# penn-graphics-research/claymore

Hardware: AMD Instinct MI355X
Metric: particles*steps/sec (higher is better)
Workload: dtype f32

## Files before the change

claymore_amd/_ffi.py:

```python
import ctypes as C
import os

MPM_OK, MPM_ERR_INVALID, MPM_ERR_DEVICE, MPM_ERR_CAPACITY, MPM_ERR_NONFINITE, MPM_ERR_NOT_READY, MPM_ERR_INTERNAL = range(7)
J_FLUID, FIXED_COROTATED, SAND, NACC = range(4)
MATERIAL_NAMES = {"jfluid": J_FLUID, "fixed_corotated": FIXED_COROTATED, "sand": SAND, "nacc": NACC}


class Config(C.Structure):
    _fields_ = [("domain_bits", C.c_int), ("max_ppc", C.c_int), ("boundary_blocks", C.c_int),
                ("gravity", C.c_float), ("cfl", C.c_float), ("max_blocks", C.c_int64),
                ("grow", C.c_int), ("drop_overflow", C.c_int), ("sync_interval", C.c_int), ("reserved", C.c_int * 3)]


class MaterialParams(C.Structure):
    _fields_ = [("rho", C.c_float), ("volume", C.c_float), ("youngs_modulus", C.c_float),
                ("poisson_ratio", C.c_float), ("bulk", C.c_float), ("gamma", C.c_float),
                ("viscosity", C.c_float), ("beta", C.c_float), ("xi", C.c_float),
                ("cohesion", C.c_float), ("yield_surface", C.c_float), ("msqr", C.c_float),
                ("log_jp0", C.c_float), ("volume_correction", C.c_int), ("hardening_on", C.c_int),
                ("reserved", C.c_int * 5)]


class CollisionObject(C.Structure):
    _fields_ = [("type", C.c_int), ("friction", C.c_float), ("scale", C.c_float), ("dsdt", C.c_float),
                ("trans", C.c_float * 3), ("trans_vel", C.c_float * 3), ("omega", C.c_float * 3),
                ("rot_mat", C.c_float * 9), ("time", C.c_float), ("reserved", C.c_int * 3)]
# ... 12 lines not shown
class Heightfield(C.Structure):
    _fields_ = [("nx", C.c_int), ("nz", C.c_int), ("origin", C.c_float * 2), ("spacing", C.c_float), ("inside_out", C.c_int),
                ("reserved", C.c_int * 6)]


HEIGHTFIELD_MAX_SAMPLES = 4096


class Counts(C.Structure):
    _fields_ = [("particle_blocks", C.c_int), ("neighbor_blocks", C.c_int), ("exterior_blocks", C.c_int),
                ("model_count", C.c_int), ("bins", C.c_int64 * 8), ("particles", C.c_int64 * 8)]


class Diagnostics(C.Structure):
    _fields_ = [("lost_particles", C.c_int64), ("discarded_p2g", C.c_int64), ("overflow_flags", C.c_int),
                ("dropped_particles", C.c_int), ("reserved", C.c_int * 4)]


class Timers(C.Structure):
    _fields_ = [("grid_update_ms", C.c_float), ("g2p2g_ms", C.c_float), ("partition_ms", C.c_float),
                ("halo_ms", C.c_float), ("total_ms", C.c_float), ("reserved", C.c_float * 3)]


_P = C.POINTER
_vp, _i, _f, _sz = C.c_void_p, C.c_int, C.c_float, C.c_size_t
_fp, _ip = _P(C.c_float), _P(C.c_int)

SIGNATURES = {
    "default_config": (_i, [_i, _P(Config)]),
    "default_material": (_i, [_i, _i, _P(MaterialParams)]),
    "create": (_i, [_P(Config), _i, _P(_vp)]),
# ... 114 lines not shown
```

claymore_amd/csrc/claymore_hip.hip:

```cpp
#include <hip/hip_runtime.h>

#include <algorithm>
#include <cmath>
#include <cstdio>
#include <cstdlib>
#include <chrono>
#include <cstring>
#include <string>
#include <vector>

#include "../../include/claymore_amd.h"
#include "mpm_kernels.hpp"
#include "mpm_readout.hpp"
#include "mpm_particle_ids.hpp"

using namespace mpm;

namespace {
constexpr int kHaloWords	 = 128;
constexpr int kStatusBlock = ST_WORDS + kHaloWords + kMaxVelSlots * kMaxVelStride;

struct Partition {
	int* table = nullptr;
	int* keys  = nullptr;
// ... 35 lines not shown
struct mpm_ctx {
	mpm_config cfg {};
	GridCfg g {};
	int device = 0;
	hipStream_t s_compute = nullptr, s_comm = nullptr;
	SubstepEvents ev;
	hipEvent_t ev_comm = nullptr, ev_halo = nullptr;
	hipEvent_t ev_tag0 = nullptr, ev_tag1 = nullptr;
	bool lean_events = false;
	hipEvent_t ev_pending = nullptr;
	hipEvent_t ev_status = nullptr;
	bool grid_preupdated = false;
	bool grid_momentum = false;
	float preupdate_dt	 = 0.f;
	float fuse_dt_once	 = 0.f;
	bool rebuild_cleared = false;
	std::vector<hipEvent_t> ev_ring;
	Partition part[2];
	float* grid[2] = {nullptr, nullptr};
	int rollid	   = 0;
	int pbc = 0, nbc = 0, ebc = 0;
	int pbc_prev = 0;
	std::vector<Model> models;
	int* d_status		  = nullptr;
	int* h_status		  = nullptr;
	unsigned* d_maxvel	  = nullptr;
	float* h_maxvel		  = nullptr;
	double* d_totals	  = nullptr;
	unsigned long long* d_counter = nullptr;
	bool ready = false;
// ... 375 lines not shown
	HIP_TRY(hipStreamSynchronize(s));
	if(pbc > g.cap) return fail(ctx, MPM_ERR_CAPACITY, "Too much active blocks: " + std::to_string(pbc));
	ctx->pbc = pbc;
	if(ctx->cfg.max_blocks <= 0 && (size_t) pbc * 27 > prov) {
		int* keys		  = nullptr;
		const size_t need = std::min(table, (size_t) pbc * 27 + 1);
		HIP_TRY(dalloc(&keys, 3 * need));
		HIP_TRY(hipMemcpyAsync(keys, P.keys, sizeof(int) * 3 * (size_t) pbc, hipMemcpyDeviceToDevice, s));
		HIP_TRY(hipStreamSynchronize(s));
		HIP_TRY(hipFree(P.keys));
		P.keys = keys;
		prov   = need;
		g.cap  = (int) prov;
	}
	HIP_TRY(hipMemcpyAsync(&ctx->d_status[ST_CNT_P], P.count, sizeof(int), hipMemcpyDeviceToDevice, s));
	register_blocks_kernel<0, 1><<<std::max(1u, std::min(4096u, cdiv((size_t) pbc * 8, 256))), 256, 0, s>>>(g, &ctx->d_status[ST_CNT_P], nullptr, &ctx->d_status[ST_CNT_N], &ctx->d_status[ST_PBC], P.table, P.keys, ctx->d_status);
	register_blocks_kernel<-1, 1><<<std::max(1u, std::min(8192u, cdiv((size_t) pbc * 32, 256))), 256, 0, s>>>(g, &ctx->d_status[ST_CNT_P], &ctx->d_status[ST_CNT_N], &ctx->d_status[ST_CNT_E], &ctx->d_status[ST_NBC], P.table, P.keys, ctx->d_status);
	{
		int rc0 = read_status(ctx);
		if(rc0) return rc0;
		rc0 = check_status(ctx);
		if(rc0) return rc0;
		const int ebc0 = ctx->h_status[ST_CNT_P] + ctx->h_status[ST_CNT_N] + ctx->h_status[ST_CNT_E];
		ctx->h_status[ST_EBC] = ebc0;
		ctx->pbc_prev		  = pbc;
		HIP_TRY(hipMemcpyAsync(&ctx->d_status[ST_EBC], &ctx->h_status[ST_EBC], sizeof(int), hipMemcpyHostToDevice, s));
		HIP_TRY(hipMemcpyAsync(&ctx->d_status[ST_PBCPREV], &ctx->pbc_prev, sizeof(int), hipMemcpyHostToDevice, s));
		HIP_TRY(hipMemcpyAsync(P.count, &ctx->h_status[ST_EBC], sizeof(int), hipMemcpyHostToDevice, s));
		HIP_TRY(hipStreamSynchronize(s));
	}
	ctx->nbc = ctx->h_status[ST_NBC];
	ctx->ebc = ctx->h_status[ST_EBC];
// ... 51 lines not shown
		ctx->models[mi].bincount_src = ctx->models[mi].bincount;
		ctx->models[mi].bucketed = (int64_t) ctx->models[mi].n;
		if((size_t) ctx->models[mi].bincount > ctx->models[mi].bin_cap) return fail(ctx, MPM_ERR_CAPACITY, "bin capacity");
	}
	HIP_TRY(hipMemcpyAsync(ctx->part[r].table, P.table, sizeof(int) * table, hipMemcpyDeviceToDevice, s));
	HIP_TRY(hipMemcpyAsync(ctx->part[r].keys, P.keys, sizeof(int) * 3 * (size_t) ctx->ebc, hipMemcpyDeviceToDevice, s));
	HIP_TRY(hipMemcpyAsync(ctx->part[r].count, P.count, sizeof(int), hipMemcpyDeviceToDevice, s));
	HIP_TRY(hipMemsetAsync(ctx->grid[0], 0, sizeof(float) * 256 * (size_t) ctx->nbc, s));
	for(auto& m: ctx->models)
		if(m.n && pbc) rasterize_blocks_kernel<<<pbc, 256, 0, s>>>(g, m.d_xyz, m.list[1], m.size, ctx->part[r].keys, ctx->part[r].table, ctx->grid[0], m.mc.mass, m.v0[0], m.v0[1], m.v0[2]);
	rc = launch_prepare(ctx, r, n, false, r, &ctx->d_status[ST_PBC], ctx->pbc, true, false);
	if(rc) return rc;
	HIP_TRY(hipGetLastError());
	HIP_TRY(hipStreamSynchronize(s));
	ctx->ready		   = true;
	ctx->grid_momentum = true;
	ctx->ids_valid	   = ctx->track_ids;
	return MPM_OK;
}

static CollisionArgs collision_tick(mpm_ctx* ctx, float dt) {
	CollisionArgs a {ctx->collision, collision_pose(ctx->collision, ctx->collision.time)};
	if(ctx->collision_running) ctx->collision.time = ctx->collision.time + dt;
	return a;
}
static ShapeArgs shapes_tick(mpm_ctx* ctx, float dt) {
	ShapeArgs a {};
	const float T = ctx->collision.time;
	a.count		  = ctx->shape_count;
	a.has_field	  = ctx->has_collision ? 1 : 0;
// ... 172 lines not shown
	PrepareModels pm {};
	pm.n = (int) ctx->models.size();
	for(int mi = 0; mi < pm.n; ++mi) {
		Model& m		  = ctx->models[mi];
		pm.list[mi]		  = m.list[list_is_out ? (m.list_in ^ 1) : m.list_in];
		pm.size[mi]		  = m.size;
		pm.row_of[mi]	  = m.row_of;
		pm.binoff_src[mi] = m.binoff[binoff_sel];
		pm.blockinfo[mi]  = m.blockinfo;
		pm.keep[mi]		  = sort && list_is_out ? m.keep : nullptr;
		pm.pairinfo[mi]	  = m.pair ? m.pairinfo[0] : nullptr;
		pm.pairhand[mi]	  = m.pairinfo[1];
	}
	const int nwg = std::max(1, std::min(ctx->g.cap, nblocks_est + nblocks_est / 16 + 64));
	int* pub	  = publish ? ctx->d_status : nullptr;
	if(sort)
		prepare_blocks_kernel<true><<<nwg, 64, 0, ctx->s_compute>>>(ctx->g, pm, pbc_ptr, ctx->part[cur].table, ctx->part[cur].keys, ctx->part[prev].table, pub, ctx->part[cur].count);
	else
		prepare_blocks_kernel<false><<<nwg, 64, 0, ctx->s_compute>>>(ctx->g, pm, pbc_ptr, ctx->part[cur].table, ctx->part[cur].keys, ctx->part[prev].table, pub, ctx->part[cur].count);
	return MPM_OK;
}

static int launch_rebuild_prepare(mpm_ctx* ctx) {
	const int r = ctx->rollid, n = r ^ 1;
	const int ebc_est = std::min(ctx->g.cap, ctx->ebc + ctx->ebc / 16 + 1024);
	return launch_prepare(ctx, n, r, true, n, &ctx->d_status[ST_CNT_P], ebc_est, true, true);
}
static int launch_rebuild(mpm_ctx* ctx, float fuse_dt = 0.f, bool without_prepare = false) {
	if(fuse_dt == 0.f) fuse_dt = ctx->fuse_dt_once;
	ctx->fuse_dt_once = 0.f;
	hipStream_t s = ctx->s_compute;
	GridCfg& g	  = ctx->g;
	const int r = ctx->rollid, n = r ^ 1;
	Partition& Pn = ctx->part[n];
	Partition& Pr = ctx->part[r];
	const bool fused = fuse_dt > 0.f;
	ctx->grid_momentum = !fused;
	int rc			 = launch_clear(ctx, kClearRebuild | (fused ? kClearMaxVel : 0));
	if(rc) return rc;
	RebuildModels rm {};
	rm.n = (int) ctx->models.size();
	for(int mi = 0; mi < rm.n; ++mi) {
		Model& m		 = ctx->models[mi];
		rm.out_count[mi] = m.out_count;
		rm.size[mi]		 = m.size;
		rm.row_of[mi]	 = m.row_of;
		rm.binoff[mi]	 = m.binoff[r];
		rm.bin_cap[mi]	 = (long long) m.bin_cap;
	}
	int* st			  = ctx->d_status;
	const int ebc_est = std::min(g.cap, ctx->ebc + ctx->ebc / 16 + 1024);
	compact_blocks_kernel<<<std::max(1u, cdiv(ebc_est, 1024)), 1024, 0, s>>>(g, rm, Pr.keys, Pn.keys, Pn.table, st);
	const unsigned rg8 = std::max(1u, std::min(4096u, cdiv((size_t) ebc_est * 8, 256))), rg32 = std::max(1u, std::min(8192u, cdiv((size_t) ebc_est * 32, 256)));
	register_blocks_kernel<0, 1><<<rg8, 256, 0, s>>>(g, &st[ST_CNT_P], nullptr, &st[ST_CNT_N], &st[ST_PBC], Pn.table, Pn.keys, st);
	if(fused) {
		if(ctx->hf_count)
			carry_grid_terrain_kernel<<<2048, 256, 0, s>>>(g, st, Pn.keys, Pr.table, ctx->grid[1], ctx->grid[0], fuse_dt, ctx->d_maxvel, terrain_tick(ctx, fuse_dt));
		else if(ctx->shape_count)
			carry_grid_shapes_kernel<<<2048, 256, 0, s>>>(g, st, Pn.keys, Pr.table, ctx->grid[1], ctx->grid[0], fuse_dt, ctx->d_maxvel, shapes_tick(ctx, fuse_dt));
		else if(ctx->has_collision)
			carry_grid_kernel<true, true><<<2048, 256, 0, s>>>(g, st, Pn.keys, Pr.table, ctx->grid[1], ctx->grid[0], fuse_dt, ctx->d_maxvel, collision_tick(ctx, fuse_dt));
		else
			carry_grid_kernel<true><<<2048, 256, 0, s>>>(g, st, Pn.keys, Pr.table, ctx->grid[1], ctx->grid[0], fuse_dt, ctx->d_maxvel, NoCollision {});
		ctx->grid_preupdated = true;
		ctx->preupdate_dt	 = fuse_dt;
	} else
		carry_grid_kernel<false><<<2048, 256, 0, s>>>(g, st, Pn.keys, Pr.table, ctx->grid[1], ctx->grid[0], 0.f, nullptr, NoCollision {});
	register_blocks_kernel<-1, 1><<<rg32, 256, 0, s>>>(g, &st[ST_CNT_P], &st[ST_CNT_N], &st[ST_CNT_E], &st[ST_NBC], Pn.table, Pn.keys, st);
	if(without_prepare) return MPM_OK;
	return launch_prepare(ctx, n, r, true, n, &st[ST_CNT_P], ebc_est, true, true);
}

static int grow_capacity(mpm_ctx* ctx) {
	if(!ctx->cfg.grow) return MPM_OK;
	hipStream_t s	   = ctx->s_compute;
	const size_t table = (size_t) ctx->g.G * ctx->g.G * ctx->g.G;
	const size_t cap   = (size_t) ctx->g.cap;
	if((size_t) ctx->ebc * 4 > cap * 3 && cap < table) {
		const size_t ncap = std::min(table, cap * 3 / 2 + 1);
		HIP_TRY(hipDeviceSynchronize());
		for(int i = 0; i < 2; ++i) {
			HIP_TRY(regrow(&ctx->part[i].keys, 3 * cap, 3 * ncap, s));
			HIP_TRY(regrow(&ctx->grid[i], cap * 256, ncap * 256, s));
// ... 7 lines not shown
			HIP_TRY(regrow(&m.row_of, cap + 1, ncap + 1, s));
			HIP_TRY(regrow(&m.out_count, cap + 1, ncap + 1, s));
			HIP_TRY(regrow(&m.keep, cap + 1, ncap + 1, s));
			HIP_TRY(regrow(&m.blockinfo, cap * (size_t) kInfoRow, ncap * (size_t) kInfoRow, s));
			if(m.pair)
				for(int i = 0; i < 2; ++i) HIP_TRY(regrow(&m.pairinfo[i], (cap + 1) * (size_t) kPairChunks, (ncap + 1) * (size_t) kPairChunks, s));
		}
		if(ctx->d_overlap) {
			HIP_TRY(regrow(&ctx->d_overlap, cap + 1, ncap + 1, s));
			HIP_TRY(regrow(&ctx->d_halo_list, cap + 1, ncap + 1, s));
			HIP_TRY(regrow(&ctx->d_inner_list, cap + 1, ncap + 1, s));
		}
		for(int p = 0; p < 32; ++p)
			if(ctx->d_send_ids[p]) HIP_TRY(regrow(&ctx->d_send_ids[p], cap + 1, ncap + 1, s));
		ctx->g.cap = (int) ncap;
		ctx->capacity_events++;
	}
	for(auto& m: ctx->models) {
		const size_t need = m.n / kBin + (size_t) ctx->g.cap + 1;
		if((size_t) m.bincount * 4 > m.bin_cap * 3 || need > m.bin_cap) {
			const size_t nb = std::max(need, (size_t) m.bincount * 4 > m.bin_cap * 3 ? m.bin_cap * 3 / 2 + 1 : m.bin_cap);
			HIP_TRY(hipDeviceSynchronize());
			for(int i = 0; i < 2; ++i) HIP_TRY(regrow(&m.bins[i], m.bin_cap * m.nch * kBin, nb * m.nch * kBin, s));
			if(ctx->track_ids)
				for(int i = 0; i < 2; ++i) HIP_TRY(regrow(&m.ids[i], m.bin_cap * kBin, nb * kBin, s));
			m.bin_cap = nb;
			ctx->capacity_events++;
		}
	}
	return MPM_OK;
}

static void roll_partition(mpm_ctx* ctx) {
	for(auto& m: ctx->models) m.list_in ^= 1;
	ctx->rollid ^= 1;
}

static int check_books(mpm_ctx* ctx) {
	const long long gone = (long long) ctx->h_status[ST_LOST] + (long long) ctx->h_status[ST_DROPPED] + ctx->books_bias;
	long long added = 0, held = 0;
	for(size_t mi = 0; mi < ctx->models.size(); ++mi) {
// ... 88 lines not shown
	HIP_TRY(hipEventElapsedTime(&ctx->last_g2p2g_ms, ctx->ev.g2p2g_start, ctx->ev.g2p2g_end));
	HIP_TRY(hipEventElapsedTime(&ctx->timers.partition_ms, ctx->ev.start, ctx->ev.end));
	ctx->timers.g2p2g_ms = ctx->last_g2p2g_ms;
	ctx->timers.total_ms = ctx->timers.grid_update_ms + ctx->timers.g2p2g_ms + ctx->timers.partition_ms;
	guard.armed = false;
	return MPM_OK;
}

int mpm_run_fixed(mpm_ctx* ctx, int nsteps, float dt) {
	phase_call(ctx);
	if(!ctx || !ctx->ready) return MPM_ERR_NOT_READY;
	HIP_TRY(hipSetDevice(ctx->device));
	hipStream_t s = ctx->s_compute;
	const int K = ctx->cfg.sync_interval > 0 ? std::min(ctx->cfg.sync_interval, 64) : 8;
	FlagGuard guard {ctx};
	while((int) ctx->ev_ring.size() < 3 * K + 1) {
		hipEvent_t e = nullptr;
		HIP_TRY(hipEventCreate(&e));
		ctx->ev_ring.push_back(e);
	}
	{
		int rc = grow_capacity(ctx);
		if(rc) return rc;
	}
	double acc_grid = 0, acc_g2p2g = 0, acc_part = 0, acc_total = 0;
	int in_window = 0;
	for(int it = 0; it < nsteps; ++it) {
		hipEvent_t* ev = &ctx->ev_ring[3 * in_window];
		if(in_window == 0) HIP_TRY(hipEventRecord(ev[0], s));
		int rc = launch_grid_update(ctx, dt);
		if(rc) return rc;
		const bool fuse_next = it + 1 < nsteps;
		rc = launch_g2p2g(ctx, dt, dt, ev[1], ev[2], true, fuse_next);
		if(rc) return rc;
		rc = launch_rebuild(ctx, fuse_next ? dt : 0.f);
		if(rc) return rc;
		HIP_TRY(hipEventRecord(ev[3], s));
		roll_partition(ctx);
		++in_window;
		const bool tight = ctx->cfg.grow && (long long) ctx->ebc * 10 > (long long) ctx->g.cap * 7 &&
						   (size_t) ctx->g.cap < (size_t) ctx->g.G * ctx->g.G * ctx->g.G;
		if(in_window == K || it + 1 == nsteps || tight) {
			HIP_TRY(hipGetLastError());
			rc = sync_counts(ctx, nullptr);
			if(rc) return rc;
			if(std::isinf(host_maxvel(ctx))) return fail(ctx, MPM_ERR_NONFINITE, "Maximum velocity is infinity");
			for(int w = 0; w < in_window; ++w) {
				hipEvent_t* e = &ctx->ev_ring[3 * w];
				float t_grid = 0, t_g = 0, t_part = 0, t_tot = 0;
				HIP_TRY(hipEventElapsedTime(&t_grid, e[0], e[1]));
// ... 259 lines not shown
	if(!ctx || !ctx->ready) return MPM_ERR_NOT_READY;
	if(block_capacity) *block_capacity = ctx->g.cap;
	if(bin_capacity)
		for(size_t i = 0; i < ctx->models.size() && i < 8; ++i) bin_capacity[i] = (int64_t) ctx->models[i].bin_cap;
	if(growth_events) *growth_events = ctx->capacity_events;
	return MPM_OK;
}

int mpm_get_diagnostics(mpm_ctx* ctx, mpm_diagnostics* d) {
	if(!ctx || !ctx->ready || !d) return MPM_ERR_NOT_READY;
	memset(d, 0, sizeof(*d));
	d->lost_particles = ctx->h_status[ST_LOST];
	d->discarded_p2g  = ctx->h_status[ST_ARENA];
	d->overflow_flags = ctx->h_status[ST_OVERFLOW];
	d->dropped_particles = ctx->h_status[ST_DROPPED];
#ifdef MPM_G2P2G_STATS
	for(int i = 0; i < 4; ++i) d->reserved[i] = ctx->h_status[24 + i];
#endif
	return MPM_OK;
}

int mpm_get_timers(mpm_ctx* ctx, mpm_timers* t) {
	if(!ctx || !t) return MPM_ERR_INVALID;
	*t = ctx->timers;
	return MPM_OK;
}

static void launch_readout(mpm_ctx* ctx, const Model& m, ReadoutKind kind, const ReadoutOut& out, hipStream_t s) {
	if(!ctx->pbc) return;
	const ReadoutArgs a = make_readout_args(ctx, m);
	switch(kind) {
	case kReadState: readout_kernel<kReadState><<<ctx->pbc, kReadoutThreads, 0, s>>>(a, nullptr, out); break;
	case kReadVelocity: readout_kernel<kReadVelocity><<<ctx->pbc, kReadoutThreads, 0, s>>>(a, ctx->grid[0], out); break;
	case kReadMomentum: readout_kernel<kReadMomentum><<<ctx->pbc, kReadoutThreads, 0, s>>>(a, ctx->grid[0], out); break;
	case kReadStress: readout_kernel<kReadStress><<<ctx->pbc, kReadoutThreads, 0, s>>>(a, nullptr, out); break;
	case kReadStressTotals: readout_kernel<kReadStressTotals><<<ctx->pbc, kReadoutThreads, 0, s>>>(a, nullptr, out); break;
	case kReadIds: readout_kernel<kReadIds><<<ctx->pbc, kReadoutThreads, 0, s>>>(a, nullptr, out); break;
	}
}
// ... 334 lines not shown
```

claymore_amd/csrc/mpm_checkpoint.inc:

```

namespace {
struct CkptModel {
	int32_t material, nch, list_in, layout;
	int64_t n, bincount, bincount_src, bucketed;
};
struct CkptHeader {
	uint64_t magic;
	int32_t domain_bits, max_ppc, nmodels, rollid;
	int32_t pbc, nbc, ebc, prev_count;
	uint64_t total_bytes;
	uint64_t param_hash;
	int32_t prev_pbc;
	int32_t grid_velocity;
	CkptModel models[8];
};
constexpr uint64_t kCkptMagic = 0x3754504b434d504dull;

struct CkptLayout {
	size_t cur_keys, prev_keys, grid, end;
	size_t size[8], row_of[8], binoff_src[8], binoff_dst[8], bins[8], lists[8], pairinfo[8];
};
static CkptLayout ckpt_layout(const CkptHeader& h) {
	CkptLayout L {};
	size_t o	= sizeof(CkptHeader);
// ... 334 lines not shown
		{
			long long added = 0, held = 0;
			for(int mi = 0; mi < h.nmodels; ++mi) added += (long long) h.models[mi].n, held += (long long) h.models[mi].bucketed;
			ctx->books_bias = added - held - ((long long) st[ST_LOST] + (long long) st[ST_DROPPED]);
		}
		HIP_TRY(hipMemcpyAsync(ctx->d_status, st, sizeof(int) * ST_WORDS, hipMemcpyHostToDevice, s));
		HIP_TRY(hipMemsetAsync(ctx->d_maxvel, 0, sizeof(unsigned) * kMaxVelSlots * kMaxVelStride, s));
	}
	{
		int rc = launch_prepare(ctx, r, n, false, r, &ctx->d_status[ST_PBC], h.pbc, false, false);
		if(rc) return rc;
	}
	HIP_TRY(hipGetLastError());
	HIP_TRY(hipStreamSynchronize(s));
	ctx->halo_tagged = false;
	ctx->ids_valid	 = false;
	return MPM_OK;
}
```

claymore_amd/csrc/mpm_g2p2g.hpp:

```cpp
#pragma once
#include "mpm_device_math.hpp"
#include "mpm_cube_lane.hpp"

namespace mpm {

constexpr int kG2P2GWaves = 3;
constexpr int kG2P2GWavesFluid = 4;

constexpr int kP2GStrideX = 36, kP2GStrideY = 6, kP2GNodes = 216;
constexpr int kP2GArena2 = 228;
constexpr int kG2PStrideX = 6, kG2PStrideY = 1, kG2PStrideZ = 36, kG2PNodes = 216;

struct ModelView {
	const float* bins_src;
	float* bins_dst;
	const int* binoff_src;
	const int* binoff_dst;
	const int* list_in;
	int* list_out;
	const int* size;
	const int* row_of;
	int* out_count;
	int* keep;
	const int* blockinfo;
// ... 557 lines not shown
			stay_rank	= lane;
			const int n_act = __popcll(__ballot(active));
			if(lane == 0) raw_stay = atomicAdd(&mv.out_count[b_opaque], n_act);
		} else {
			const bool dir_ok = ((unsigned) (dirv[0] + 1) < 3u) & ((unsigned) (dirv[1] + 1) < 3u) & ((unsigned) (dirv[2] + 1) < 3u);
			ntag			  = dir_ok ? (dirv[0] + 1) * 9 + (dirv[1] + 1) * 3 + dirv[2] + 1 : kStay;
			const int dno_raw = __shfl(info, 27 + ntag);
			dno				  = (active && dir_ok) ? dno_raw : -1;
			stay			  = dno >= 0 && ntag == kStay;
			const unsigned long long stay_m = __ballot(stay);
			stay_leader						= stay_m ? __ffsll((long long) stay_m) - 1 : 0;
			stay_rank						= (int) __builtin_amdgcn_mbcnt_hi((unsigned) (stay_m >> 32), __builtin_amdgcn_mbcnt_lo((unsigned) stay_m, 0u));
			if(stay_m != 0ull && lane == stay_leader) raw_stay = atomicAdd(&mv.out_count[b_opaque], __popcll(stay_m));
			if(dno >= 0 && !stay) raw_move = atomicAdd(&mv.out_count[dno], 1);
			if(active) {
				if(dno < 0) atomicAdd(&status[ST_LOST], 1);
				if(!in_arena) atomicAdd(&status[ST_ARENA], 1);
			}
		}
		chain.template at<1>();
		const int pkey = pk[1] * 36 + pk[0] * 6 + pk[2];
		const int rec  = (ntag << tag_shift) | (pkey << key_shift) | pidib;
		settled		   = settled && __all(!active || (stay && pkey == okey));
		chain.template at<2>();
		MPM_MARK("L_material");
		float* dbin = mv.bins_dst + (size_t) (binoff_dst + (pidib >> 6)) * (kBin * NCH);
		float4* dst = reinterpret_cast<float4*>(dbin + (pidib & 63) * REC);
		if constexpr(MAT == 0) {
			chain.template at<kPreSites + 0>();
			const float J = stress_jfluid(mv.mc, sk.ss.vol, sk.jdiv, sk.jvisc, st[0], A, pl.contrib);
// ... 112 lines not shown
```

claymore_amd/csrc/mpm_g2p2g_pair.hpp:

```cpp
#pragma once
#include "mpm_g2p2g.hpp"

namespace mpm {

struct ChainHalf {
	float pw[3][3];
	float cx0, cy0, cz0;
	v2f_ cx12, cy12, cz12;
	float slab0, pen0, wij;
	v2f_ slab12, pen12;
	MPM_DEV void init(const P2GPayload& p, bool on) {
#pragma unroll
		for(int d = 0; d < 3; ++d) bspline_weight_cells(p.fd[d], pw[d]);
		if(!on) pw[0][0] = pw[0][1] = pw[0][2] = 0.f;
		cx0	 = p.contrib[0], cy0 = p.contrib[3], cz0 = p.contrib[6];
		cx12 = (v2f_) {p.contrib[1], p.contrib[2]}, cy12 = (v2f_) {p.contrib[4], p.contrib[5]}, cz12 = (v2f_) {p.contrib[7], p.contrib[8]};
		slab0  = p.mv[0] - cx0 * p.fd[0] - cy0 * p.fd[1] - cz0 * p.fd[2];
		slab12 = (v2f_) {p.mv[1], p.mv[2]} - cx12 * p.fd[0] - cy12 * p.fd[1] - cz12 * p.fd[2];
	}
	MPM_DEV void prep(int o, float mass, float& W, v2f_& m0, v2f_& t12) {
		const int i = o / 9, j = (o / 3) % 3, k = o % 3;
		if(k == 0) {
			if(j == 0) {
				if(i != 0) {
// ... 281 lines not shown
				ntag[h]			  = dir_ok ? (dirv[h][0] + 1) * 9 + (dirv[h][1] + 1) * 3 + dirv[h][2] + 1 : kStay;
				const int dno_raw = __shfl(info, 27 + ntag[h]);
				dno[h]			  = (active[h] && dir_ok) ? dno_raw : -1;
				stay[h]			  = dno[h] >= 0 && ntag[h] == kStay;
				stay_m[h]		  = __ballot(stay[h]);
				stay_rank[h]	  = (int) __builtin_amdgcn_mbcnt_hi((unsigned) (stay_m[h] >> 32), __builtin_amdgcn_mbcnt_lo((unsigned) stay_m[h], 0u));
			}
			stay_rank[1] += __popcll(stay_m[0]);
			const unsigned long long any_m = stay_m[0] | stay_m[1];
			stay_leader					   = any_m ? __ffsll((long long) any_m) - 1 : 0;
			if(any_m != 0ull && lane == stay_leader) raw_stay = atomicAdd(&mv.out_count[b_opaque], __popcll(stay_m[0]) + __popcll(stay_m[1]));
#pragma unroll
			for(int h = 0; h < 2; ++h) {
				if(dno[h] >= 0 && !stay[h]) raw_move[h] = atomicAdd(&mv.out_count[dno[h]], 1);
				if(active[h]) {
					if(dno[h] < 0) atomicAdd(&status[ST_LOST], 1);
					if(!in_arena[h]) atomicAdd(&status[ST_ARENA], 1);
				}
			}
		}
		int pkey[2], rec[2];
#pragma unroll
		for(int h = 0; h < 2; ++h) {
			pkey[h] = pk[h][1] * 36 + pk[h][0] * 6 + pk[h][2];
			rec[h]	= (ntag[h] << tag_shift) | (pkey[h] << key_shift) | pidib[h] | (arena_sel << kArenaBit);
		}
		settled = settled && __all((!active[0] || (stay[0] && pkey[0] == okey[0])) && (!active[1] || (stay[1] && pkey[1] == okey[1])));
		MPM_MARK("P_material");
		float contrib[2][9];
		NoHook nohook;
// ... 140 lines not shown
```

claymore_amd/csrc/mpm_kernels.hpp:

```cpp
#pragma once
#include <hip/hip_runtime.h>
#include <type_traits>

#include "mpm_device_math.hpp"
#include "mpm_collision.hpp"
#include "mpm_collision_shapes.hpp"
#include "mpm_collision_heightfield.hpp"

namespace mpm {

constexpr int kBin		  = 64;
constexpr int kG2P2GThreads = 64;
constexpr int kMaxModels  = 8;
constexpr int kSortKeys		= 216;
constexpr int kKeyBits		= 8;
constexpr int kStay		  = 13;

enum {
	ST_PBC = 0, ST_NBC = 1, ST_EBC = 2, ST_OVERFLOW = 3, ST_LOST = 4, ST_ARENA = 5, ST_DROPPED = 6, ST_NONFINITE = 7, ST_BINS0 = 8, ST_PART0 = 16,
	 ST_CNT_P = 29, ST_CNT_N = 30, ST_CNT_E = 31, ST_BINSPREV = 32, ST_PBCPREV = 40, ST_WORDS = 64
};

struct GridCfg {
	int G;
	int gbits;
	int ppb;
	int pid_bits;
	int boundary;
	int cap;
	float dx, dx_inv, d_inv, gravity;
};

__device__ __forceinline__ bool key_ok(const GridCfg& c, int x, int y, int z) {
	return ((unsigned) x < (unsigned) c.G) & ((unsigned) y < (unsigned) c.G) & ((unsigned) z < (unsigned) c.G);
}
__device__ __forceinline__ size_t key_index(const GridCfg& c, int x, int y, int z) {
// ... 407 lines not shown
}

constexpr int kInfoRow = 64;
struct PrepareModels {
	int n;
	int* list[kMaxModels];
	const int* size[kMaxModels];
	const int* row_of[kMaxModels];
	const int* binoff_src[kMaxModels];
	int* blockinfo[kMaxModels];
	const int* keep[kMaxModels];
	int* pairinfo[kMaxModels];
	const int* pairhand[kMaxModels];
};
template<bool SORT>
__global__ __launch_bounds__(64) void prepare_blocks_kernel(GridCfg cfg, PrepareModels pm, const int* __restrict__ pbc_ptr, const int* __restrict__ cur_table, const int* __restrict__ cur_keys, const int* __restrict__ prev_table, int* __restrict__ publish, int* __restrict__ part_count) {
	constexpr int kPrepChunk = kListChunk;
	__shared__ int s_sorted[kPairChunkMax];
	__shared__ int s_cnt[256];
	__shared__ int s_cur[256];
	const int lane = threadIdx.x;
	if(publish && blockIdx.x == 0 && lane == 0) {
		const int ebc	 = publish[ST_CNT_P] + publish[ST_CNT_N] + publish[ST_CNT_E];
		publish[ST_EBC] = ebc;
		*part_count		 = ebc;
	}
	const int pbc = min(*pbc_ptr, cfg.cap);
	for(int b = blockIdx.x; b < pbc; b += gridDim.x) {
	const int kx = cur_keys[3 * b], ky = cur_keys[3 * b + 1], kz = cur_keys[3 * b + 2];
	int size0 = 0, row0 = 0, keep0 = -2, hand0 = 0;
	if constexpr(SORT) {
		if(pm.n > 0) {
			size0 = pm.size[0][b];
			row0  = pm.row_of[0][b];
			if(pm.keep[0]) keep0 = pm.keep[0][row0];
			if(pm.pairinfo[0]) hand0 = pm.pairhand[0][(size_t) row0 * kPairChunks + (lane & (kPairChunks - 1))];
		}
	}
	int srcno = -1, other = -1;
	if(lane < 27) {
		int ox, oy, oz;
		dir_components(lane, ox, oy, oz);
		srcno = table_query(cfg, prev_table, kx + ox, ky + oy, kz + oz);
	} else if(lane < 54) {
		int ox, oy, oz;
		dir_components(lane - 27, ox, oy, oz);
		other = table_query(cfg, cur_table, kx - ox, ky - oy, kz - oz);
	} else if(lane < 62) {
		const int lb = lane - 54;
		other		 = table_query(cfg, cur_table, kx + ((lb >> 2) & 1), ky + ((lb >> 1) & 1), kz + (lb & 1));
	}
	const int key_shift		= cfg.pid_bits;
	const int tag_shift		= cfg.pid_bits + kKeyBits;
	const unsigned rec_mask = (1u << (tag_shift + 5)) - 1u;
	for(int m = 0; m < pm.n; ++m) {
// ... 177 lines not shown
			const int left = size - chunk0;
			const int nrec = (pairinfo && left > kPrepChunk && left <= kPairChunkMax) ? left : min(kPrepChunk, left);
			if(chunk0) load_chunk(chunk0, min(kPrepChunk, nrec));
			if(pairinfo)
				sort_chunk_pairs(chunk0, nrec);
			else
				sort_chunk(chunk0, nrec);
			if(nrec > kPrepChunk) break;
		}
		}
		if constexpr(!SORT) {
			if(lane < 27) info = srcno >= 0 ? pm.binoff_src[m][srcno] : -1;
		}
		pm.blockinfo[m][(size_t) b * kInfoRow + lane] = info;
	}
	}
}

}
#include "mpm_g2p2g.hpp"
#include "mpm_g2p2g_pair.hpp"
namespace mpm {

struct RebuildModels {
	int n;
	const int* out_count[kMaxModels];
	int* size[kMaxModels];
	int* row_of[kMaxModels];
	int* binoff[kMaxModels];
	long long bin_cap[kMaxModels];
};

enum { kClearP2G = 1, kClearRebuild = 2, kClearMaxVel = 4 };
struct ClearArgs {
	int flags;
	int nmodels;
	int* out_count[kMaxModels];
	int* keep[kMaxModels];
	float* p2g_grid;
	int* status;
	unsigned* max_vel_bits;
	int* old_table;
	const int* old_keys;
	const int* old_count;
};
__global__ __launch_bounds__(256) void substep_clear_kernel(GridCfg cfg, ClearArgs a) {
	const int tid = blockIdx.x * 256 + threadIdx.x, nthreads = gridDim.x * 256;
	if(a.flags & kClearP2G) {
		const int nbc = min(a.status[ST_NBC], cfg.cap), ebc = min(a.status[ST_EBC], cfg.cap);
		float4* g	  = reinterpret_cast<float4*>(a.p2g_grid);
		for(int i = tid; i < nbc * 64; i += nthreads) g[i] = make_float4(0.f, 0.f, 0.f, 0.f);
		for(int m = 0; m < a.nmodels; ++m)
			for(int i = tid; i <= ebc; i += nthreads) a.out_count[m][i] = 0, a.keep[m][i] = -1;
	}
	if(a.flags & kClearRebuild) {
		const int n = min(*a.old_count, cfg.cap);
		for(int i = tid; i < n; i += nthreads) a.old_table[key_index(cfg, a.old_keys[3 * i], a.old_keys[3 * i + 1], a.old_keys[3 * i + 2])] = -1;
		if(blockIdx.x == gridDim.x - 1) {
			if(threadIdx.x < kMaxModels) {
				a.status[ST_BINSPREV + threadIdx.x] = a.status[ST_BINS0 + threadIdx.x];
				a.status[ST_BINS0 + threadIdx.x]	= 0;
				a.status[ST_PART0 + threadIdx.x]	= 0;
			}
			if(threadIdx.x >= 8 && threadIdx.x < 11) a.status[ST_CNT_P + threadIdx.x - 8] = 0;
			if(threadIdx.x == 11) a.status[ST_PBCPREV] = a.status[ST_PBC];
			if(threadIdx.x >= 64 && threadIdx.x < 64 + kMaxVelSlots) {
				unsigned* slot = a.max_vel_bits + (threadIdx.x - 64) * kMaxVelStride;
				if(*slot >= 0x7f800000u) a.status[ST_NONFINITE] = 1;
				if(a.flags & kClearMaxVel) *slot = 0u;
			}
		}
	}
}

__global__ __launch_bounds__(1024) void compact_blocks_kernel(GridCfg cfg, RebuildModels rm, const int* __restrict__ old_keys, int* __restrict__ new_keys, int* __restrict__ new_table, int* __restrict__ status) {
	__shared__ int s_part[kMaxModels];
	const int ebc = min(status[ST_EBC], cfg.cap);
	for(int b0 = blockIdx.x * blockDim.x; b0 < ebc; b0 += gridDim.x * blockDim.x) {
		const int b = b0 + threadIdx.x;
		int c[kMaxModels];
		bool any = false;
		for(int m = 0; m < rm.n; ++m) {
			c[m] = b < ebc ? rm.out_count[m][b] : 0;
			if(c[m] > cfg.ppb) {
				atomicAdd(&status[ST_DROPPED], c[m] - cfg.ppb);
				c[m] = cfg.ppb;
			}
			any |= c[m] > 0;
		}
		__syncthreads();
		if(threadIdx.x < kMaxModels) s_part[threadIdx.x] = 0;
		__syncthreads();
		for(int m = 0; m < rm.n; ++m) {
			int t = c[m];
#pragma unroll
			for(int off = 32; off > 0; off >>= 1) t += __shfl_xor(t, off);
			if((threadIdx.x & 63) == 0 && t) atomicAdd(&s_part[m], t);
		}
		__syncthreads();
		if((int) threadIdx.x < rm.n && s_part[threadIdx.x]) atomicAdd(&status[ST_PART0 + threadIdx.x], s_part[threadIdx.x]);
		const int nb = block_append(&status[ST_CNT_P], any ? 1 : 0);
		int kx = 0, ky = 0, kz = 0;
		if(any) {
			kx = old_keys[3 * b], ky = old_keys[3 * b + 1], kz = old_keys[3 * b + 2];
			new_keys[3 * nb]					  = kx;
			new_keys[3 * nb + 1]				  = ky;
			new_keys[3 * nb + 2]				  = kz;
			new_table[key_index(cfg, kx, ky, kz)] = nb;
		}
		for(int m = 0; m < rm.n; ++m) {
			const int nbins = any ? (c[m] + kBin - 1) / kBin : 0;
			const int first = block_append(&status[ST_BINS0 + m], nbins);
			if(any) {
				const bool fits = (long long) first + nbins <= rm.bin_cap[m];
				if(!fits) atomicOr(&status[ST_OVERFLOW], 4);
				rm.size[m][nb]	 = fits ? c[m] : 0;
				rm.row_of[m][nb] = b;
				rm.binoff[m][nb] = (nbins && fits) ? first : 0;
			}
		}
	}
}

template<int LO, int HI>
__global__ __launch_bounds__(256) void register_blocks_kernel(GridCfg cfg, const int* __restrict__ pbc_ptr, const int* __restrict__ base2_ptr, int* counter, int* publish, int* table, int* keys, int* status) {
	constexpr int W	   = HI - LO + 1;
	constexpr int NOFF = W * W * W;
	constexpr int LPB  = NOFF <= 8 ? 8 : 32;
	const int pbc	   = min(*pbc_ptr, cfg.cap);
	const int base	   = *pbc_ptr + (base2_ptr ? *base2_ptr : 0);
	if(publish && blockIdx.x == 0 && threadIdx.x == 0) *publish = base;
	const long long total = (long long) pbc * LPB;
	const long long bound = (total + blockDim.x - 1) / blockDim.x * blockDim.x;
	for(long long t = (long long) blockIdx.x * blockDim.x + threadIdx.x; t < bound; t += (long long) gridDim.x * blockDim.x) {
		const int b = (int) (t / LPB), o = (int) (t % LPB);
		bool claim	= false;
		int x = 0, y = 0, z = 0;
		size_t i = 0;
		if(t < total && o < NOFF) {
			x = keys[3 * b] + LO + o / (W * W);
			y = keys[3 * b + 1] + LO + (o / W) % W;
			z = keys[3 * b + 2] + LO + o % W;
			if(key_ok(cfg, x, y, z)) {
				i = key_index(cfg, x, y, z);
				if(table[i] == -1) claim = atomicCAS(&table[i], -1, -2) == -1;
			}
// ... 283 lines not shown
```

include/claymore_amd.h:

```cpp
#ifndef CLAYMORE_AMD_H
#define CLAYMORE_AMD_H

#include <stddef.h>
#include <stdint.h>

#ifdef __cplusplus
extern "C" {
#endif

typedef enum mpm_status {
	MPM_OK			   = 0,
	MPM_ERR_INVALID	   = 1,
	MPM_ERR_DEVICE	   = 2,
	MPM_ERR_CAPACITY   = 3,
	MPM_ERR_NONFINITE  = 4,
	MPM_ERR_NOT_READY  = 5,
	MPM_ERR_INTERNAL   = 6
} mpm_status;

typedef enum mpm_material {
	MPM_J_FLUID			= 0,
	MPM_FIXED_COROTATED = 1,
	MPM_SAND			= 2,
	MPM_NACC			= 3
} mpm_material;

typedef struct mpm_config {
	int domain_bits;
	int max_ppc;
	int boundary_blocks;
	float gravity;
	float cfl;
	int64_t max_blocks;
	int grow;
	int drop_overflow;
	int sync_interval;
	int reserved[3];
} mpm_config;

typedef struct mpm_material_params {
	float rho;
	float volume;
	float youngs_modulus;
	float poisson_ratio;
	float bulk;
	float gamma;
	float viscosity;
	float beta;
	float xi;
	float cohesion;
	float yield_surface;
	float msqr;
// ... 100 lines not shown
	float origin[2];
	float spacing;
	int inside_out;
	int reserved[6];
} mpm_heightfield;
int mpm_set_collision_heightfield(mpm_ctx* ctx, int slot, const mpm_collision_object* obj, const mpm_heightfield* hf, const float* heights);
int mpm_test_collision_heightfield(const mpm_collision_object* obj, const mpm_heightfield* hf, const float* heights, float time, const float* xyz, size_t n, float* out4, int device);

int mpm_get_capacity(mpm_ctx* ctx, int64_t* block_capacity, int64_t* bin_capacity, int* growth_events);
int mpm_get_timers(mpm_ctx* ctx, mpm_timers* t);
typedef struct mpm_diagnostics {
	int64_t lost_particles;
	int64_t discarded_p2g;
	int overflow_flags;
	int dropped_particles;
	int reserved[4];
} mpm_diagnostics;
int mpm_get_diagnostics(mpm_ctx* ctx, mpm_diagnostics* d);
int mpm_grid_totals(mpm_ctx* ctx, double out[4]);
int mpm_check_table(mpm_ctx* ctx);
int mpm_dump_grid(mpm_ctx* ctx, int* keys, float* blocks, size_t* nblocks);
const char* mpm_build_info(void);
int mpm_last_g2p2g_ms(mpm_ctx* ctx, float* ms);

int mpm_test_eig(const float* F, size_t n, float* out12, int device);
int mpm_test_stress(int material, const mpm_material_params* p, const float* F, const float* logjp, size_t n, float* out19, int device);

int mpm_halo_keys(mpm_ctx* ctx, int* dev_keys, int capacity_blocks, int* count);
int mpm_halo_tag_begin(mpm_ctx* ctx);
int mpm_halo_tag_peer(mpm_ctx* ctx, int peer, const int* dev_peer_keys, int npeer_keys);
int mpm_halo_tag_end(mpm_ctx* ctx, int* halo_particle_blocks, int* send_counts);
// ... 35 lines not shown
```

Baseline: 35.60 billion.

## Skip partition rebuild work when no particle changed blocks

G2P2G now sets a device-side moved flag whenever any active particle leaves its block. When the flag stays clear, the rebuild reuses the previous block layout: it copies keys and table entries, skips both register_blocks passes, and lets prepare_blocks derive neighbour info from existing blockinfo rows, or skip already-complete blocks after a streak of such steps. This targets the per-step partition rebuild cost in run_fixed. The trade-off is an extra global store in the particle loop, more branching in the rebuild kernels, and reliance on the relaid flag to invalidate the cache after regrowth, setup or checkpoint load. It also adds a waves-per-EU hint on prepare_blocks.

```diff
diff --git a/claymore_amd/_ffi.py b/claymore_amd/_ffi.py
--- a/claymore_amd/_ffi.py
+++ b/claymore_amd/_ffi.py
@@ -9,7 +9,8 @@
 class Config(C.Structure):
     _fields_ = [("domain_bits", C.c_int), ("max_ppc", C.c_int), ("boundary_blocks", C.c_int),
                 ("gravity", C.c_float), ("cfl", C.c_float), ("max_blocks", C.c_int64),
-                ("grow", C.c_int), ("drop_overflow", C.c_int), ("sync_interval", C.c_int), ("reserved", C.c_int * 3)]
+                ("grow", C.c_int), ("drop_overflow", C.c_int), ("sync_interval", C.c_int), ("still_rebuild", C.c_int),
+                ("reserved", C.c_int * 2)]
 
 
 class MaterialParams(C.Structure):
@@ -52,7 +53,7 @@
 
 class Diagnostics(C.Structure):
     _fields_ = [("lost_particles", C.c_int64), ("discarded_p2g", C.c_int64), ("overflow_flags", C.c_int),
-                ("dropped_particles", C.c_int), ("reserved", C.c_int * 4)]
+                ("dropped_particles", C.c_int), ("reserved", C.c_int * 3), ("still_rebuilds", C.c_int)]
 
 
 class Timers(C.Structure):
diff --git a/claymore_amd/csrc/claymore_hip.hip b/claymore_amd/csrc/claymore_hip.hip
--- a/claymore_amd/csrc/claymore_hip.hip
+++ b/claymore_amd/csrc/claymore_hip.hip
@@ -73,6 +73,8 @@
 	bool grid_momentum = false;
 	float preupdate_dt	 = 0.f;
 	float fuse_dt_once	 = 0.f;
+	bool relaid = true;
+	int allow_still = 0;
 	bool rebuild_cleared = false;
 	std::vector<hipEvent_t> ev_ring;
 	Partition part[2];
@@ -478,8 +480,8 @@
 		g.cap  = (int) prov;
 	}
 	HIP_TRY(hipMemcpyAsync(&ctx->d_status[ST_CNT_P], P.count, sizeof(int), hipMemcpyDeviceToDevice, s));
-	register_blocks_kernel<0, 1><<<std::max(1u, std::min(4096u, cdiv((size_t) pbc * 8, 256))), 256, 0, s>>>(g, &ctx->d_status[ST_CNT_P], nullptr, &ctx->d_status[ST_CNT_N], &ctx->d_status[ST_PBC], P.table, P.keys, ctx->d_status);
-	register_blocks_kernel<-1, 1><<<std::max(1u, std::min(8192u, cdiv((size_t) pbc * 32, 256))), 256, 0, s>>>(g, &ctx->d_status[ST_CNT_P], &ctx->d_status[ST_CNT_N], &ctx->d_status[ST_CNT_E], &ctx->d_status[ST_NBC], P.table, P.keys, ctx->d_status);
+	register_blocks_kernel<0, 1><<<std::max(1u, std::min(4096u, cdiv((size_t) pbc * 8, 256))), 256, 0, s>>>(g, &ctx->d_status[ST_CNT_P], nullptr, &ctx->d_status[ST_CNT_N], &ctx->d_status[ST_PBC], P.table, P.keys, ctx->d_status, 0);
+	register_blocks_kernel<-1, 1><<<std::max(1u, std::min(8192u, cdiv((size_t) pbc * 32, 256))), 256, 0, s>>>(g, &ctx->d_status[ST_CNT_P], &ctx->d_status[ST_CNT_N], &ctx->d_status[ST_CNT_E], &ctx->d_status[ST_NBC], P.table, P.keys, ctx->d_status, 0);
 	{
 		int rc0 = read_status(ctx);
 		if(rc0) return rc0;
@@ -561,6 +563,7 @@
 	HIP_TRY(hipGetLastError());
 	HIP_TRY(hipStreamSynchronize(s));
 	ctx->ready		   = true;
+	ctx->relaid		   = true;
 	ctx->grid_momentum = true;
 	ctx->ids_valid	   = ctx->track_ids;
 	return MPM_OK;
@@ -763,10 +766,11 @@
 	}
 	const int nwg = std::max(1, std::min(ctx->g.cap, nblocks_est + nblocks_est / 16 + 64));
 	int* pub	  = publish ? ctx->d_status : nullptr;
+	const int still = publish && sort && list_is_out ? ctx->allow_still : 0;
 	if(sort)
-		prepare_blocks_kernel<true><<<nwg, 64, 0, ctx->s_compute>>>(ctx->g, pm, pbc_ptr, ctx->part[cur].table, ctx->part[cur].keys, ctx->part[prev].table, pub, ctx->part[cur].count);
+		prepare_blocks_kernel<true><<<nwg, 64, 0, ctx->s_compute>>>(ctx->g, pm, pbc_ptr, ctx->part[cur].table, ctx->part[cur].keys, ctx->part[prev].table, pub, ctx->part[cur].count, still);
 	else
-		prepare_blocks_kernel<false><<<nwg, 64, 0, ctx->s_compute>>>(ctx->g, pm, pbc_ptr, ctx->part[cur].table, ctx->part[cur].keys, ctx->part[prev].table, pub, ctx->part[cur].count);
+		prepare_blocks_kernel<false><<<nwg, 64, 0, ctx->s_compute>>>(ctx->g, pm, pbc_ptr, ctx->part[cur].table, ctx->part[cur].keys, ctx->part[prev].table, pub, ctx->part[cur].count, still);
 	return MPM_OK;
 }
 
@@ -775,7 +779,7 @@
 	const int ebc_est = std::min(ctx->g.cap, ctx->ebc + ctx->ebc / 16 + 1024);
 	return launch_prepare(ctx, n, r, true, n, &ctx->d_status[ST_CNT_P], ebc_est, true, true);
 }
-static int launch_rebuild(mpm_ctx* ctx, float fuse_dt = 0.f, bool without_prepare = false) {
+static int launch_rebuild(mpm_ctx* ctx, float fuse_dt = 0.f, bool without_prepare = false, bool allow_still = false) {
 	if(fuse_dt == 0.f) fuse_dt = ctx->fuse_dt_once;
 	ctx->fuse_dt_once = 0.f;
 	hipStream_t s = ctx->s_compute;
@@ -784,6 +788,9 @@
 	Partition& Pn = ctx->part[n];
 	Partition& Pr = ctx->part[r];
 	const bool fused = fuse_dt > 0.f;
+	const int still	 = allow_still && !ctx->relaid ? 1 : 0;
+	ctx->allow_still = still;
+	ctx->relaid		 = false;
 	ctx->grid_momentum = !fused;
 	int rc			 = launch_clear(ctx, kClearRebuild | (fused ? kClearMaxVel : 0));
 	if(rc) return rc;
@@ -795,13 +802,14 @@
 		rm.size[mi]		 = m.size;
 		rm.row_of[mi]	 = m.row_of;
 		rm.binoff[mi]	 = m.binoff[r];
+		rm.binoff_cur[mi] = m.binoff[n];
 		rm.bin_cap[mi]	 = (long long) m.bin_cap;
 	}
 	int* st			  = ctx->d_status;
 	const int ebc_est = std::min(g.cap, ctx->ebc + ctx->ebc / 16 + 1024);
-	compact_blocks_kernel<<<std::max(1u, cdiv(ebc_est, 1024)), 1024, 0, s>>>(g, rm, Pr.keys, Pn.keys, Pn.table, st);
+	compact_blocks_kernel<<<std::max(1u, cdiv(ebc_est, 1024)), 1024, 0, s>>>(g, rm, Pr.keys, Pn.keys, Pn.table, st, still);
 	const unsigned rg8 = std::max(1u, std::min(4096u, cdiv((size_t) ebc_est * 8, 256))), rg32 = std::max(1u, std::min(8192u, cdiv((size_t) ebc_est * 32, 256)));
-	register_blocks_kernel<0, 1><<<rg8, 256, 0, s>>>(g, &st[ST_CNT_P], nullptr, &st[ST_CNT_N], &st[ST_PBC], Pn.table, Pn.keys, st);
+	register_blocks_kernel<0, 1><<<rg8, 256, 0, s>>>(g, &st[ST_CNT_P], nullptr, &st[ST_CNT_N], &st[ST_PBC], Pn.table, Pn.keys, st, still);
 	if(fused) {
 		if(ctx->hf_count)
 			carry_grid_terrain_kernel<<<2048, 256, 0, s>>>(g, st, Pn.keys, Pr.table, ctx->grid[1], ctx->grid[0], fuse_dt, ctx->d_maxvel, terrain_tick(ctx, fuse_dt));
@@ -815,7 +823,7 @@
 		ctx->preupdate_dt	 = fuse_dt;
 	} else
 		carry_grid_kernel<false><<<2048, 256, 0, s>>>(g, st, Pn.keys, Pr.table, ctx->grid[1], ctx->grid[0], 0.f, nullptr, NoCollision {});
-	register_blocks_kernel<-1, 1><<<rg32, 256, 0, s>>>(g, &st[ST_CNT_P], &st[ST_CNT_N], &st[ST_CNT_E], &st[ST_NBC], Pn.table, Pn.keys, st);
+	register_blocks_kernel<-1, 1><<<rg32, 256, 0, s>>>(g, &st[ST_CNT_P], &st[ST_CNT_N], &st[ST_CNT_E], &st[ST_NBC], Pn.table, Pn.keys, st, still);
 	if(without_prepare) return MPM_OK;
 	return launch_prepare(ctx, n, r, true, n, &st[ST_CNT_P], ebc_est, true, true);
 }
@@ -853,6 +861,7 @@
 		for(int p = 0; p < 32; ++p)
 			if(ctx->d_send_ids[p]) HIP_TRY(regrow(&ctx->d_send_ids[p], cap + 1, ncap + 1, s));
 		ctx->g.cap = (int) ncap;
+		ctx->relaid = true;
 		ctx->capacity_events++;
 	}
 	for(auto& m: ctx->models) {
@@ -864,6 +873,7 @@
 			if(ctx->track_ids)
 				for(int i = 0; i < 2; ++i) HIP_TRY(regrow(&m.ids[i], m.bin_cap * kBin, nb * kBin, s));
 			m.bin_cap = nb;
+			ctx->relaid = true;
 			ctx->capacity_events++;
 		}
 	}
@@ -982,6 +992,7 @@
 	hipStream_t s = ctx->s_compute;
 	const int K = ctx->cfg.sync_interval > 0 ? std::min(ctx->cfg.sync_interval, 64) : 8;
 	FlagGuard guard {ctx};
+	const bool still_on = ctx->cfg.still_rebuild != -1 && ctx->group_refs == 0;
 	while((int) ctx->ev_ring.size() < 3 * K + 1) {
 		hipEvent_t e = nullptr;
 		HIP_TRY(hipEventCreate(&e));
@@ -1001,7 +1012,7 @@
 		const bool fuse_next = it + 1 < nsteps;
 		rc = launch_g2p2g(ctx, dt, dt, ev[1], ev[2], true, fuse_next);
 		if(rc) return rc;
-		rc = launch_rebuild(ctx, fuse_next ? dt : 0.f);
+		rc = launch_rebuild(ctx, fuse_next ? dt : 0.f, false, still_on);
 		if(rc) return rc;
 		HIP_TRY(hipEventRecord(ev[3], s));
 		roll_partition(ctx);
@@ -1291,8 +1302,9 @@
 	d->discarded_p2g  = ctx->h_status[ST_ARENA];
 	d->overflow_flags = ctx->h_status[ST_OVERFLOW];
 	d->dropped_particles = ctx->h_status[ST_DROPPED];
+	d->still_rebuilds	 = ctx->h_status[ST_STILL];
 #ifdef MPM_G2P2G_STATS
-	for(int i = 0; i < 4; ++i) d->reserved[i] = ctx->h_status[24 + i];
+	for(int i = 0; i < 3; ++i) d->reserved[i] = ctx->h_status[24 + i];
 #endif
 	return MPM_OK;
 }
@@ -1300,6 +1312,9 @@
 int mpm_get_timers(mpm_ctx* ctx, mpm_timers* t) {
 	if(!ctx || !t) return MPM_ERR_INVALID;
 	*t = ctx->timers;
+#ifdef MPM_G2P2G_STATS
+	if(ctx->h_status) memcpy(&t->reserved[0], &ctx->h_status[27], sizeof(int));
+#endif
 	return MPM_OK;
 }
 
diff --git a/claymore_amd/csrc/mpm_checkpoint.inc b/claymore_amd/csrc/mpm_checkpoint.inc
--- a/claymore_amd/csrc/mpm_checkpoint.inc
+++ b/claymore_amd/csrc/mpm_checkpoint.inc
@@ -372,6 +372,7 @@
 	HIP_TRY(hipGetLastError());
 	HIP_TRY(hipStreamSynchronize(s));
 	ctx->halo_tagged = false;
+	ctx->relaid		 = true;
 	ctx->ids_valid	 = false;
 	return MPM_OK;
 }
diff --git a/claymore_amd/csrc/mpm_g2p2g.hpp b/claymore_amd/csrc/mpm_g2p2g.hpp
--- a/claymore_amd/csrc/mpm_g2p2g.hpp
+++ b/claymore_amd/csrc/mpm_g2p2g.hpp
@@ -595,6 +595,7 @@
 			if(stay_m != 0ull && lane == stay_leader) raw_stay = atomicAdd(&mv.out_count[b_opaque], __popcll(stay_m));
 			if(dno >= 0 && !stay) raw_move = atomicAdd(&mv.out_count[dno], 1);
 			if(active) {
+				if(!stay) status[ST_MOVED] = 1;
 				if(dno < 0) atomicAdd(&status[ST_LOST], 1);
 				if(!in_arena) atomicAdd(&status[ST_ARENA], 1);
 			}
diff --git a/claymore_amd/csrc/mpm_g2p2g_pair.hpp b/claymore_amd/csrc/mpm_g2p2g_pair.hpp
--- a/claymore_amd/csrc/mpm_g2p2g_pair.hpp
+++ b/claymore_amd/csrc/mpm_g2p2g_pair.hpp
@@ -319,6 +319,7 @@
 			for(int h = 0; h < 2; ++h) {
 				if(dno[h] >= 0 && !stay[h]) raw_move[h] = atomicAdd(&mv.out_count[dno[h]], 1);
 				if(active[h]) {
+					if(!stay[h]) status[ST_MOVED] = 1;
 					if(dno[h] < 0) atomicAdd(&status[ST_LOST], 1);
 					if(!in_arena[h]) atomicAdd(&status[ST_ARENA], 1);
 				}
diff --git a/claymore_amd/csrc/mpm_kernels.hpp b/claymore_amd/csrc/mpm_kernels.hpp
--- a/claymore_amd/csrc/mpm_kernels.hpp
+++ b/claymore_amd/csrc/mpm_kernels.hpp
@@ -18,8 +18,15 @@
 
 enum {
 	ST_PBC = 0, ST_NBC = 1, ST_EBC = 2, ST_OVERFLOW = 3, ST_LOST = 4, ST_ARENA = 5, ST_DROPPED = 6, ST_NONFINITE = 7, ST_BINS0 = 8, ST_PART0 = 16,
-	 ST_CNT_P = 29, ST_CNT_N = 30, ST_CNT_E = 31, ST_BINSPREV = 32, ST_PBCPREV = 40, ST_WORDS = 64
+	 ST_CNT_P = 29, ST_CNT_N = 30, ST_CNT_E = 31, ST_BINSPREV = 32, ST_PBCPREV = 40,
+	ST_MOVED = 42,
+	ST_STILL = 43,
+	ST_STREAK = 44,
+	ST_WORDS = 64
 };
+__device__ __forceinline__ bool rebuild_is_still(int allow_still, const int* status) {
+	return allow_still && status[ST_MOVED] == 0;
+}
 
 struct GridCfg {
 	int G;
@@ -457,7 +464,7 @@
 	const int* pairhand[kMaxModels];
 };
 template<bool SORT>
-__global__ __launch_bounds__(64) void prepare_blocks_kernel(GridCfg cfg, PrepareModels pm, const int* __restrict__ pbc_ptr, const int* __restrict__ cur_table, const int* __restrict__ cur_keys, const int* __restrict__ prev_table, int* __restrict__ publish, int* __restrict__ part_count) {
+__global__ __launch_bounds__(64) __attribute__((amdgpu_waves_per_eu(6))) void prepare_blocks_kernel(GridCfg cfg, PrepareModels pm, const int* __restrict__ pbc_ptr, const int* __restrict__ cur_table, const int* __restrict__ cur_keys, const int* __restrict__ prev_table, int* __restrict__ publish, int* __restrict__ part_count, int allow_still) {
 	constexpr int kPrepChunk = kListChunk;
 	__shared__ int s_sorted[kPairChunkMax];
 	__shared__ int s_cnt[256];
@@ -469,8 +476,11 @@
 		*part_count		 = ebc;
 	}
 	const int pbc = min(*pbc_ptr, cfg.cap);
-	for(int b = blockIdx.x; b < pbc; b += gridDim.x) {
-	const int kx = cur_keys[3 * b], ky = cur_keys[3 * b + 1], kz = cur_keys[3 * b + 2];
+	const bool still = rebuild_is_still(allow_still, publish);
+	const bool skip = still && publish[ST_STREAK] >= 2;
+	auto prepare_block = [&](const int b) {
+	int kx = 0, ky = 0, kz = 0;
+	if(!still) kx = cur_keys[3 * b], ky = cur_keys[3 * b + 1], kz = cur_keys[3 * b + 2];
 	int size0 = 0, row0 = 0, keep0 = -2, hand0 = 0;
 	if constexpr(SORT) {
 		if(pm.n > 0) {
@@ -481,7 +491,14 @@
 		}
 	}
 	int srcno = -1, other = -1;
-	if(lane < 27) {
+	if(still) {
+		const int stand	 = pm.n > 0 ? pm.blockinfo[0][(size_t) b * kInfoRow + lane] : -1;
+		const int mirror = __shfl(stand, (53 - lane) & 63);
+		if(lane < 27)
+			srcno = mirror;
+		else if(lane < 62)
+			other = stand;
+	} else if(lane < 27) {
 		int ox, oy, oz;
 		dir_components(lane, ox, oy, oz);
 		srcno = table_query(cfg, prev_table, kx + ox, ky + oy, kz + oz);
@@ -689,7 +706,21 @@
 		}
 		pm.blockinfo[m][(size_t) b * kInfoRow + lane] = info;
 	}
-	}
+	};
+	if(skip) {
+		for(long long base = (long long) blockIdx.x * 64; base < pbc; base += (long long) gridDim.x * 64) {
+			const int c = (int) base + lane;
+			bool done	= true;
+			if(c < pbc)
+				for(int m = 0; m < pm.n; ++m) {
+					const int size = pm.size[m][c], tail = size & (kPrepChunk - 1);
+					done = done && (size == 0 || (pm.keep[m][c] == size && (pm.pairinfo[m] || tail <= 64 || (tail & 63) == 0)));
+				}
+			for(unsigned long long todo = __ballot(!done); todo != 0ull; todo &= todo - 1ull) prepare_block((int) base + __ffsll((long long) todo) - 1);
+		}
+		return;
+	}
+	for(int b = blockIdx.x; b < pbc; b += gridDim.x) prepare_block(b);
 }
 
 }
@@ -703,6 +734,7 @@
 	int* size[kMaxModels];
 	int* row_of[kMaxModels];
 	int* binoff[kMaxModels];
+	const int* binoff_cur[kMaxModels];
 	long long bin_cap[kMaxModels];
 };
 
@@ -725,6 +757,7 @@
 		const int nbc = min(a.status[ST_NBC], cfg.cap), ebc = min(a.status[ST_EBC], cfg.cap);
 		float4* g	  = reinterpret_cast<float4*>(a.p2g_grid);
 		for(int i = tid; i < nbc * 64; i += nthreads) g[i] = make_float4(0.f, 0.f, 0.f, 0.f);
+		if(tid == 0) a.status[ST_MOVED] = 0;
 		for(int m = 0; m < a.nmodels; ++m)
 			for(int i = tid; i <= ebc; i += nthreads) a.out_count[m][i] = 0, a.keep[m][i] = -1;
 	}
@@ -748,9 +781,23 @@
 	}
 }
 
-__global__ __launch_bounds__(1024) void compact_blocks_kernel(GridCfg cfg, RebuildModels rm, const int* __restrict__ old_keys, int* __restrict__ new_keys, int* __restrict__ new_table, int* __restrict__ status) {
+__global__ __launch_bounds__(1024) void compact_blocks_kernel(GridCfg cfg, RebuildModels rm, const int* __restrict__ old_keys, int* __restrict__ new_keys, int* __restrict__ new_table, int* __restrict__ status, int allow_still) {
 	__shared__ int s_part[kMaxModels];
 	const int ebc = min(status[ST_EBC], cfg.cap);
+	const bool still = rebuild_is_still(allow_still, status);
+	const int pbc	 = min(status[ST_PBC], cfg.cap);
+	if(still && blockIdx.x == 0) {
+		if(threadIdx.x < kMaxModels) status[ST_BINS0 + threadIdx.x] = status[ST_BINSPREV + threadIdx.x];
+		if(threadIdx.x == 64) {
+			const int p = status[ST_PBC], n = status[ST_NBC];
+			status[ST_CNT_P] = p;
+			status[ST_CNT_N] = n - p;
+			status[ST_CNT_E] = status[ST_EBC] - n;
+			status[ST_STILL] += 1;
+			status[ST_STREAK] += 1;
+		}
+	} else if(blockIdx.x == 0 && threadIdx.x == 64)
+		status[ST_STREAK] = 0;
 	for(int b0 = blockIdx.x * blockDim.x; b0 < ebc; b0 += gridDim.x * blockDim.x) {
 		const int b = b0 + threadIdx.x;
 		int c[kMaxModels];
@@ -774,6 +821,22 @@
 		}
 		__syncthreads();
 		if((int) threadIdx.x < rm.n && s_part[threadIdx.x]) atomicAdd(&status[ST_PART0 + threadIdx.x], s_part[threadIdx.x]);
+		if(still) {
+			if(b < ebc) {
+				const int kx = old_keys[3 * b], ky = old_keys[3 * b + 1], kz = old_keys[3 * b + 2];
+				new_keys[3 * b]						  = kx;
+				new_keys[3 * b + 1]					  = ky;
+				new_keys[3 * b + 2]					  = kz;
+				new_table[key_index(cfg, kx, ky, kz)] = b;
+				if(b < pbc)
+					for(int m = 0; m < rm.n; ++m) {
+						rm.size[m][b]	= c[m];
+						rm.row_of[m][b] = b;
+						rm.binoff[m][b] = rm.binoff_cur[m][b];
+					}
+			}
+			continue;
+		}
 		const int nb = block_append(&status[ST_CNT_P], any ? 1 : 0);
 		int kx = 0, ky = 0, kz = 0;
 		if(any) {
@@ -798,13 +861,14 @@
 }
 
 template<int LO, int HI>
-__global__ __launch_bounds__(256) void register_blocks_kernel(GridCfg cfg, const int* __restrict__ pbc_ptr, const int* __restrict__ base2_ptr, int* counter, int* publish, int* table, int* keys, int* status) {
+__global__ __launch_bounds__(256) void register_blocks_kernel(GridCfg cfg, const int* __restrict__ pbc_ptr, const int* __restrict__ base2_ptr, int* counter, int* publish, int* table, int* keys, int* status, int allow_still) {
 	constexpr int W	   = HI - LO + 1;
 	constexpr int NOFF = W * W * W;
 	constexpr int LPB  = NOFF <= 8 ? 8 : 32;
 	const int pbc	   = min(*pbc_ptr, cfg.cap);
 	const int base	   = *pbc_ptr + (base2_ptr ? *base2_ptr : 0);
 	if(publish && blockIdx.x == 0 && threadIdx.x == 0) *publish = base;
+	if(rebuild_is_still(allow_still, status)) return;
 	const long long total = (long long) pbc * LPB;
 	const long long bound = (total + blockDim.x - 1) / blockDim.x * blockDim.x;
 	for(long long t = (long long) blockIdx.x * blockDim.x + threadIdx.x; t < bound; t += (long long) gridDim.x * blockDim.x) {
diff --git a/include/claymore_amd.h b/include/claymore_amd.h
--- a/include/claymore_amd.h
+++ b/include/claymore_amd.h
@@ -35,7 +35,8 @@
 	int grow;
 	int drop_overflow;
 	int sync_interval;
-	int reserved[3];
+	int still_rebuild;
+	int reserved[2];
 } mpm_config;
 
 typedef struct mpm_material_params {
@@ -166,7 +167,8 @@
 	int64_t discarded_p2g;
 	int overflow_flags;
 	int dropped_particles;
-	int reserved[4];
+	int reserved[3];
+	int still_rebuilds;
 } mpm_diagnostics;
 int mpm_get_diagnostics(mpm_ctx* ctx, mpm_diagnostics* d);
 int mpm_grid_totals(mpm_ctx* ctx, double out[4]);
```

Measured after the change: 37.12 billion (median of 6 runs). 1.04x the previous value.
